# LivGen/LMAT

Measured on AMD Instinct MI355X. Metric: reads/s (150 bp) vs 64 GB k-mer DB, higher is better.
Workload: dtype u64; 1 GPU; 1104000000 x 150 bp reads/GPU vs 64 GiB k-mer hash (6467472668 20-mers, replicated per GPU), run_rl.sh flags -x 0 -j 30 -l 0 -b 1, calls-only; total_reads=1104000000, reads_per_launch=8000000, read_len=150, db_kmers=6467472668, k=20, parallelism=reads sharded x1, DB replicated, genus_block_permille=100, prune_g=0, list_replicas=1, distinct_lists=792576, reads_called=1058323347, read_pool_batches=32

## Files before the change

lmat_amd/csrc/kernels.hip:

```cpp
#include <hip/hip_runtime.h>
#include <atomic>
#include <type_traits>
#include "kernels.hpp"

#ifndef LMAT_ABLATE
#define LMAT_ABLATE 0
#endif
#define STOP_AT(n, v) do { if (LMAT_ABLATE && A.prm.stop_after == (n)) { if (lane == 0) { emit(250, (v)); } return; } } while (0)
#ifndef LMAT_CLOSURE_FAST
#define LMAT_CLOSURE_FAST 1
#endif
#ifndef LMAT_LDS_SHIFT
#define LMAT_LDS_SHIFT 0
#endif

namespace lmat {

#define WSYNC()                                              \
    do {                                                     \
        __builtin_amdgcn_fence(__ATOMIC_SEQ_CST, "wavefront"); \
        __builtin_amdgcn_wave_barrier();                     \
    } while (0)

template <bool GMEM>
// ... 1475 lines not shown
        }
        const bool done = vrow && !bail;
        uint32_t coff = 0, ncand = 0;
        if (A.cands && bal(done && !phix)) {
            uint32_t c0 = 0;
            if (done && !phix && li == 0) c0 = G_ADD(&g_cursor[0], nT);
            coff = bp(c0, 0);
            const bool room = (uint64_t)coff + nT <= A.cand_cap;
            if (done && !phix && !room && li == 0) G_OR((GAS uint32_t*)A.err, (uint32_t)kErrCandOverflow);
            if (done && !phix && room && act)
                ((GAS uint64_t*)((GAS lmat_cand*)A.cands + coff))[nT - 1u - (uint32_t)li] = (uint64_t)g_tid32[ptid] | ((uint64_t)__float_as_uint(pscore) << 32);
            if (room) ncand = nT;
        }
        if (vrow && li == 0) {
            GAS uint64_t* out = (GAS uint64_t*)(A.results + it);
            if (bail) {
                *(GAS uint8_t*)out = 254;
                ((GAS uint32_t*)A.k4_bail)[G_ADD(&g_cursor[6], 1u)] = (uint32_t)it;
            } else {
                lmat_read_result res;
                uint64_t wv[5];
                wv[0] = out[0]; wv[1] = out[1]; wv[2] = out[2]; wv[3] = out[3]; wv[4] = out[4];
                __builtin_memcpy(&res, wv, 40);
                res.cand_kmer_cnt = (uint16_t)cand;
                uint32_t call_idx;
                if (phix) {
                    res.status = LMAT_ST_PHIX; res.match_type = LMAT_MT_DIRECT; res.call_tid = 32630; res.call_score = phix_score;
                    res.log_avg = 0; res.stdev = 0; res.cand_off = 0; res.n_cand = 0;
                    call_idx = A.phix_call_idx;
                } else {
                    res.status = LMAT_ST_CALL; res.match_type = (uint8_t)match; res.log_avg = log_avg; res.stdev = stdev1;
                    res.call_tid = call_tid ? g_tid32[call_tid] : 0u; res.call_score = call_score;
                    res.cand_off = coff; res.n_cand = ncand;
                    call_idx = call_tid;
                }
                store_result(out, res);
                if (res.status != LMAT_ST_PHIX && res.match_type == LMAT_MT_NOMATCH) {
                    G_ADD(&tally_nomatch[1], 1ull);
                } else if (res.call_score >= A.prm.min_score) {
                    G_ADD(&tally_count[call_idx], 1ull);
                    G_ADD(&tally_score[call_idx], (double)res.call_score);
                } else if (res.call_score < A.prm.min_score) {
                    G_ADD(&tally_nomatch[2], 1ull);
                }
            }
        }
    }
}

#define WSYNC_WAVE WSYNC
#pragma push_macro("WSYNC")
#undef WSYNC
#define WSYNC() wsync<(U > 2048)>()
template <int LPR>
__global__ __launch_bounds__(256) void tail_kernel(ClassifyArgs A) {
    const uint64_t gi = (uint64_t)blockIdx.x * 256 + threadIdx.x;
    const uint64_t it = gi / LPR;
    const uint32_t j = (uint32_t)(gi % LPR);
    if (it >= A.count) return;
    const uint64_t r = A.index ? (uint64_t)A.index[it] : A.first + it;
    const DeviceTables& tb = A.tb;
    const int k = tb.k;
    const uint64_t off = A.rec_off[r];
    const uint32_t p = 128u + j;
    const uint32_t wb = (2 * p) >> 5, ws = (2 * p) & 31;
    const uint32_t* codes = A.words + off + 1;
    const uint32_t len = A.words[off], cr0 = codes[wb], cr1 = codes[wb + 1], cr2 = codes[wb + 2];
    if ((int)len < k) return;
    const uint32_t P = len - k + 1;
    if (P <= 128u || P > 128u + LPR) return;
    const uint32_t nb = (len + 15) / 16, nm = (len + 31) / 32;
    const uint32_t* vmask = codes + nb;
    auto cw = [&](uint32_t i) -> uint64_t { const uint32_t v = i == wb ? cr0 : (i == wb + 1 ? cr1 : cr2); return i < nb ? v : 0u; };
    auto vw = [&](uint32_t i) -> uint64_t { return i < nm ? vmask[i] : 0u; };
    const uint64_t kmask = (1ull << (2 * k)) - 1;
    const uint32_t wmask = (1u << k) - 1;
    const uint32_t mb = p >> 5, ms = p & 31;
    const uint64_t m2 = (vw(mb + 1) << 32) | vw(mb);
    const uint64_t lo = (cw(wb + 1) << 32) | cw(wb);
    uint64_t w = ws ? ((lo >> ws) | (cw(wb + 2) << (64 - ws))) : lo;
    w &= kmask;
    const uint64_t rev = (~w) & kmask;
    uint64_t f = __builtin_bitreverse64(w);
    f = ((f & 0x5555555555555555ull) << 1) | ((f >> 1) & 0x5555555555555555ull);
    f >>= (64 - 2 * k);
    const bool fc = f < rev;
    const uint64_t km = fc ? f : rev, kr = fc ? rev : f;
    const uint64_t ri = r - A.result_base;
    if (j < 3u) {
        const int cm = tb.cpt.m;
        const uint64_t x = f >> (2 * (kCptW - 1)), xr = rev & ((1ull << (2 * cm)) - 1);
        ((uint64_t*)A.tail_u)[ri * 4 + j] = (cpt_scramble(x < xr ? x : xr, cm) << 4) | (xr < x ? 2u : 0u) | (x == xr ? 1u : 0u);
    }
    u32x4 e = {0u, 0u, 0u, 0u};
    if (p < P) {
        uint32_t b, tag;
        cpt_address(*(const CptGeom*)&tb.cpt, km, kr, b, tag);
        const uint32_t jj = ((tag - 1u) >> 7) & 3u;
        const uint32_t* bk = (const uint32_t*)tb.slots + (uint64_t)b * 16;
        const u32x4 q0 = *(const u32x4*)bk, q1 = *(const u32x4*)(bk + 4), q2 = *(const u32x4*)(bk + 8), q3 = *(const u32x4*)(bk + 12);
        const uint32_t tg[6] = {q0.x, q0.y, q0.z, q0.w, q1.x, q1.y};
        const uint32_t pw[6] = {q1.z, q1.w, q2.x, q2.y, q2.z, q2.w};
        const uint32_t ph[3] = {q3.x, q3.y, q3.z};
        uint32_t pay = 0;
        bool hit = false;
#pragma unroll
        for (int i = kCptSlots - 1; i >= 0; --i) {
            const uint32_t t = (tg[i >> 1] >> (16 * (i & 1))) & 0xFFFFu;
            if (t == (tag & 0xFFFFu)) {
                hit = true;
                pay = ((pw[i >> 1] >> (16 * (i & 1))) & 0xFFFFu) | (((ph[i >> 2] >> (8 * (i & 3))) & 0xFFu) << 16);
            }
        }
        const bool valid = ((uint32_t)(m2 >> ms) & wmask) == wmask;
        if (valid) {
            if (!hit && (q3.w & kCptOvfFlag)) pay = wide_lookup(tb.ovf_slots, tb.ovf_nbuckets, ovf_bucket_of(b, tag & 0xFFFFu, tb.ovf_nbuckets), km);
            e = u32x4{(uint32_t)km, (uint32_t)(km >> 32), b, pay | (1u << 24) | ((fc ? jj : (uint32_t)(kCptW - 1) - jj) << 30)};
        }
    }
    ((u32x4*)A.tail16)[ri * LPR + j] = e;
}

typedef const ClassifyArgs __attribute__((address_space(4))) CArgs;
template <int U, int T, int E, bool INK4, bool PERM, bool CPT, bool WIDE = false, bool PLAIN = false>
__device__ __forceinline__ void classify_one(CArgs* Ap, uint64_t r, unsigned char* lds, LAS unsigned char* xl, int lane,
                                             const uint32_t* wcur, uint32_t (&nmacc)[2]) {
    using L = WL<U, T, E, INK4, CPT, WIDE>;
    constexpr int THM = L::TH - 1;
    using tid_t = typename std::conditional<WIDE, uint32_t, uint16_t>::type;
    using ent_t = typename std::conditional<WIDE, unsigned long long, unsigned int>::type;
    using lin_t = typename std::conditional<WIDE, LinEntW, LinEnt>::type;
    constexpr int ESH = WIDE ? 32 : 16;
    constexpr ent_t EIDM = WIDE ? (ent_t)0xFFFFFFFFull : (ent_t)0xFFFFu;
    constexpr uint32_t EPEND = WIDE ? 0x80000000u : 0x8000u;
#define RELANE() do { asm volatile("" : "+v"(lane)); } while (0)
#pragma push_macro("A")
#pragma push_macro("tb")
#define A (*Ap)
#define tb (Ap->tb)
    RELANE();
    uint32_t* rd = (uint32_t*)(lds + L::OFF_RD);
    unsigned long long* hv = (unsigned long long*)(lds + L::OFF_R1);
    tid_t* reg = (tid_t*)(lds + L::OFF_R1);
    uint16_t* stamp = (uint16_t*)(reg + T);
    uint16_t* cnt = stamp + T;
    uint16_t* leaf = cnt + T;
    ent_t* hent = (ent_t*)(leaf + T);
    ent_t* best = hent + L::TH;
    uint16_t* dep = (uint16_t*)(best + L::TH);
    uint16_t* ord = dep + T;
    tid_t* tin = (tid_t*)(ord + T);
    tid_t* tout = tin + T;
    float* score = (float*)(tout + T);
    uint8_t* sflags = (uint8_t*)(score + T);
    float* score0 = (float*)(sflags + T);
    float* nm_rp = score0 + T;
    uint8_t* nm_cl = (uint8_t*)(nm_rp + T);
    unsigned long long* ukmer = (unsigned long long*)(lds + L::OFF_R2);
    uint32_t* ubucket = (uint32_t*)(lds + L::OFF_R2 + 8 * U);
    uint32_t* dpay = (uint32_t*)(lds + L::OFF_R2);
    uint16_t* dmult = (uint16_t*)(lds + L::OFF_R2 + 4 * L::D);
    uint16_t* dn = dmult + L::D;
    uint16_t* dstart = dn + L::D;
    uint8_t* dfl = (uint8_t*)(dstart + L::D);
    lin_t* lin = (lin_t*)(lds + L::OFF_R2);
    uint32_t* upay = (uint32_t*)(lds + (CPT ? L::OFF_UPAY_C : L::OFF_R3));
    using eld_t = typename std::conditional<INK4, uint16_t, uint8_t>::type;
    uint32_t* el_poff = (uint32_t*)(lds + L::OFF_R3);
    tid_t* el_t = INK4 ? (tid_t*)(el_poff + E) : (tid_t*)(lds + L::OFF_R3);
    tid_t* el_ta = el_t + E;
    tid_t* el_sp = el_ta + E;
    eld_t* el_d = WIDE ? (eld_t*)(el_sp + E) : (eld_t*)(el_ta + (INK4 ? E : 2 * E));
    uint16_t* el_off = (uint16_t*)(el_ta + E);
// ... 155 lines not shown
    auto cpt_finish = [&](int c, uint64_t km, uint64_t u, uint64_t un, uint64_t fcmask, uint32_t& b_out, uint32_t& t_out) {
        const uint32_t ulo = (uint32_t)u, uhi = (uint32_t)(u >> 32);
        uint32_t u1l, u1h, u2l, u2h, u3l, u3h;
        if constexpr (LSH) {
            const LAS uint64_t* up = (const LAS uint64_t*)xl + c * 64 + lane;
            const uint64_t U1 = up[1], U2 = up[2], U3 = up[3];
            u1l = (uint32_t)U1; u1h = (uint32_t)(U1 >> 32); u2l = (uint32_t)U2; u2h = (uint32_t)(U2 >> 32); u3l = (uint32_t)U3; u3h = (uint32_t)(U3 >> 32);
        } else {
            const int n0l = __builtin_amdgcn_readlane((int)(uint32_t)un, 0), n0h = __builtin_amdgcn_readlane((int)(uint32_t)(un >> 32), 0);
            const int n1l = __builtin_amdgcn_readlane((int)(uint32_t)un, 1), n1h = __builtin_amdgcn_readlane((int)(uint32_t)(un >> 32), 1);
            const int n2l = __builtin_amdgcn_readlane((int)(uint32_t)un, 2), n2h = __builtin_amdgcn_readlane((int)(uint32_t)(un >> 32), 2);
            u1l = (uint32_t)__builtin_amdgcn_update_dpp(n0l, (int)ulo, 0x130, 0xf, 0xf, false);
            u1h = (uint32_t)__builtin_amdgcn_update_dpp(n0h, (int)uhi, 0x130, 0xf, 0xf, false);
            u2l = (uint32_t)__builtin_amdgcn_update_dpp(n1l, (int)u1l, 0x130, 0xf, 0xf, false);
            u2h = (uint32_t)__builtin_amdgcn_update_dpp(n1h, (int)u1h, 0x130, 0xf, 0xf, false);
            u3l = (uint32_t)__builtin_amdgcn_update_dpp(n2l, (int)u2l, 0x130, 0xf, 0xf, false);
            u3h = (uint32_t)__builtin_amdgcn_update_dpp(n2h, (int)u2h, 0x130, 0xf, 0xf, false);
        }
        const bool fc = lane_bit(fcmask);
        const uint32_t dirm = fc ? 0u : 12u;
        const uint64_t a0 = ((uint64_t)uhi << 32) | (ulo + dirm), a1 = ((uint64_t)u1h << 32) | (u1l + (dirm ^ 4u));
        const uint64_t a2 = ((uint64_t)u2h << 32) | (u2l + (dirm ^ 8u)), a3 = ((uint64_t)u3h << 32) | (u3l + (dirm ^ 12u));
        const uint64_t m01 = a0 < a1 ? a0 : a1, m23 = a2 < a3 ? a2 : a3;
        const uint64_t best = m01 < m23 ? m01 : m23;
        const uint32_t j = ((uint32_t)best >> 2) & 3u, fl = (uint32_t)best & 3u;
        const uint32_t strand = fc ? fl >> 1 : (fl == 0u ? 1u : 0u);
        const uint64_t sp = cpt_mix(best >> 4, cm);
        const int lb = PLAIN ? 2 : tb.cpt.lowbits;
        const uint32_t hi = (uint32_t)(sp >> lb), low = (uint32_t)sp & ((1u << lb) - 1);
        const int wsh = tb.cpt.wshift;
        uint32_t b, rho;
        if (wsh >= 0) { b = hi >> wsh; rho = hi & ((1u << wsh) - 1u); }
        else if (wsh == -2) {
            const uint32_t nb32 = (uint32_t)tb.cpt.nb, lowp = hi * nb32;
            const uint64_t nb64 = nb32;
            b = __umulhi(hi, nb32);
            rho = (lowp >= nb32 ? 1u : 0u) + ((uint64_t)lowp >= 2 * nb64 ? 1u : 0u) + ((uint64_t)lowp >= 3 * nb64 ? 1u : 0u);
        }
        else { b = (uint32_t)(((double)hi + 0.5) * tb.cpt.invW); rho = hi - b * tb.cpt.W; }
        const int rs = 2 * (kCptW - 1 - (int)j);
        const uint32_t other = (uint32_t)((km >> (2 * cm + rs)) << rs) | ((uint32_t)km & ((1u << rs) - 1));
        b_out = b;
        t_out = (1u + (((((rho << lb) | low) * 4 + j) * 2 + strand) * 64 + other)) | ((fc ? j : (uint32_t)(kCptW - 1) - j) << 30);
    };
    if (CACHE) {
#pragma unroll
        for (int c = 0; c < CH; ++c) {
            if ((uint32_t)c * 64 >= len) break;
            if (TAILOK && c == 2 && tail_mode()) {
                const uint32_t lpr = PLAIN ? 4u : A.tail_lpr;
                const uint64_t ri = r - A.result_base;
                u32x4 te = {0u, 0u, 0u, 0u};
                uint64_t tu = 0;
                if ((uint32_t)lane < lpr) te = ((const GAS u32x4*)A.tail16)[ri * lpr + lane];
                if (lane < 3) tu = ((const GAS uint64_t*)A.tail_u)[ri * 4 + lane];
                kreg[c] = ((uint64_t)(te.y & 0xFFu) << 32) | te.x;
                hreg[c] = te.z;
                treg[c] = te.w & 0xC0000000u;
                okm[c] = __ballot((te.w >> 24) & 1u);
                valid_kmers += popc64(okm[c]);
                ureg[c] = tu;
                if (128u + (uint32_t)lane < P) upay[128 + lane] = te.w & 0xFFFFFFu;
                continue;
            }
            pass1_chunk((uint32_t)c * 64, kreg[c], hreg[c], treg[c], okm[c], ureg[c], fcm[c]);
        }
        STOP_AT(47, 0);
        if (CPT) {
            if constexpr (LSH) {
                WSYNC();
                LAS uint64_t* ush = (LAS uint64_t*)xl;
#pragma unroll
                for (int c = 0; c < CH; ++c) ush[c * 64 + lane] = ureg[c];
                if (lane < 4) ush[CH * 64 + lane] = 0ull;
                WSYNC();
            }
#pragma unroll
            for (int c = 0; c < CH; ++c) {
                if ((uint32_t)c * 64 >= P) break;
                if (TAILOK && c == 2 && tail_mode()) continue;
                cpt_finish(c, kreg[c], ureg[c], c + 1 < CH ? ureg[c + 1] : 0ull, fcm[c], hreg[c], treg[c]);
            }
        }
    } else {
        for (uint32_t p0 = 0; p0 < len; p0 += 64) { uint64_t a; uint32_t b, t; uint64_t v, u, f; pass1_chunk(p0, a, b, t, v, u, f); }
    }
    WSYNC();
    if (tot > 0) {
        const float q = (float)gc / (float)tot;
        const float gc_pcnt = (float)((double)q * 100.0);
        bin_sel = __builtin_amdgcn_readfirstlane((int)(gc_pcnt / 10.0f));
    }
    if (valid_kmers < A.prm.min_kmer) {
        if (lane == 0) { emit(LMAT_ST_SHORT_VALID, 0); nmacc[0]++; }
        return;
    }
    STOP_AT(1, 0);
    RELANE();
    uint32_t nuniq = 0;
    uint32_t nscan = 0;
    if constexpr (!CPT) {
    auto pass2_chunk = [&](uint32_t p0, uint64_t km, uint32_t h, bool ok) {
        const uint32_t p = p0 + lane;
        const bool first = ok && (uint32_t)(hv[h] & 0xFFFF) == p;
        const uint64_t bm = __ballot(first);
        if (first) {
            const uint32_t rk = nuniq + prefix_count(bm);
            ukmer[rk] = (km << kPayloadBits) + 1;
// ... 1476 lines not shown
            WSYNC();
        }
        if (!done && lane == 0) {
            lmat_read_result res;
            res.status = 255; res.match_type = LMAT_MT_NOMATCH; res.cand_kmer_cnt = 0; res.valid_kmers = 0; res.read_len = 0; res.log_avg = 0;
            res.stdev = 0; res.call_tid = 0; res.call_score = 0; res.cand_off = 0; res.n_cand = 0; res.bin_sel = 0;
            store_result(out, res);
        }
    }
}

template <int LPB>
__global__ __launch_bounds__(64) void gather_bench_kernel(const uint64_t* __restrict__ slots, uint32_t nbuckets,
                                                          uint64_t probes_per_wave, uint64_t seed,
                                                          unsigned long long* sink) {
    const int lane = threadIdx.x & 63, g = lane / LPB, q = lane % LPB;
    constexpr int PPL = 64 / LPB;
    const GAS u32x4* quarters = (const GAS u32x4*)slots;
    unsigned long long acc = 0;
    uint64_t ctr = (uint64_t)blockIdx.x * probes_per_wave;
    for (uint64_t i = 0; i < probes_per_wave; i += 9 * PPL) {
        u32x4 sl[9];
#pragma unroll
        for (int j = 0; j < 9; ++j) {
            uint32_t b = bucket_of(seed + ctr + i + j * PPL + g, nbuckets);
            if (LPB == 8) b &= ~1u;
            sl[j] = quarters[(uint64_t)b * 4 + q];
        }
#pragma unroll
        for (int j = 0; j < 9; ++j) acc += (sl[j].x >> 13) + sl[j].w;
    }
    if (acc == 0x123456789ull) atomicAdd(sink, acc);
}

#pragma push_macro("WSYNC")
#undef WSYNC
#define WSYNC() wsync<(U > 2048)>()
#ifndef LMAT_FAST_WAVES
#define LMAT_FAST_WAVES 8
#endif
constexpr int classify_waves(int U, int E, bool INK4, bool CPT) { return INK4 ? 1 : (E > kFastE ? (U <= 160 ? 5 : 2) : (U <= 160 ? (CPT ? LMAT_FAST_WAVES : 5) : (U <= 256 ? (CPT ? LMAT_FAST_WAVES : 5) : (U <= 320 ? (CPT ? 5 : 3) : (CPT ? 4 : 3))))); }
template <int U, int T, int E, bool INK4, bool PERM, bool CPT, bool WIDE = false, bool PLAIN = false>
__global__ __launch_bounds__(64, classify_waves(U, E, INK4, CPT)) void classify_kernel(ClassifyArgs A) {
    extern __shared__ __align__(16) unsigned char lds_smem[];
    unsigned char* smem = U > 2048 ? A.gscratch + (size_t)blockIdx.x * WL<U, T, E, INK4, false, WIDE>::BYTES : lds_smem;
    LAS unsigned char* xl = (LAS unsigned char*)(U > 2048 ? lds_smem : lds_smem + WL<U, T, E, INK4, CPT, WIDE>::OFF_XL);
    const int lane = threadIdx.x & 63;
    constexpr int NW = (WL<U, T, E, INK4, CPT, WIDE>::RD_WORDS + 1 + 63) / 64;
    const uint32_t G = gridDim.x;
    uint32_t it = blockIdx.x;
    uint32_t wcur[NW], wnext[NW];
    uint32_t nmacc[2] = {0, 0};
    uint64_t off1 = 0;
    {
        const uint64_t count = !PLAIN && A.count_ptr ? (uint64_t)*(const GAS uint32_t*)A.count_ptr : A.count;
        if (it >= count) return;
        const GAS uint32_t* index = PLAIN ? nullptr : (const GAS uint32_t*)A.index;
        const GAS uint64_t* rec_off = (const GAS uint64_t*)A.rec_off;
        const GAS uint32_t* words = (const GAS uint32_t*)A.words;
        auto r_of = [&](uint64_t i) -> uint64_t { return index ? (uint64_t)index[i] : A.first + i; };
        const uint64_t off0 = rec_off[r_of(it)];
        off1 = (uint64_t)it + G < count ? rec_off[r_of((uint64_t)it + G)] : 0;
#pragma unroll
        for (int j = 0; j < NW; ++j) wcur[j] = words[off0 + lane + 64 * j];
    }
    while (true) {
        CArgs* Ap = (CArgs*)__builtin_amdgcn_kernarg_segment_ptr();
        asm volatile("" : "+s"(Ap));
        const uint64_t count = !PLAIN && Ap->count_ptr ? (uint64_t)*(const GAS uint32_t*)Ap->count_ptr : Ap->count;
        const GAS uint32_t* index = PLAIN ? nullptr : (const GAS uint32_t*)Ap->index;
        const GAS uint64_t* rec_off = (const GAS uint64_t*)Ap->rec_off;
        const GAS uint32_t* words = (const GAS uint32_t*)Ap->words;
        auto r_of = [&](uint64_t i) -> uint64_t { return index ? (uint64_t)index[i] : Ap->first + i; };
        const uint64_t off2 = (uint64_t)it + 2 * (uint64_t)G < count ? rec_off[r_of((uint64_t)it + 2 * (uint64_t)G)] : 0;
        const bool more = (uint64_t)it + G < count;
#pragma unroll
        for (int j = 0; j < NW; ++j) wnext[j] = more ? words[off1 + lane + 64 * j] : 0u;
        classify_one<U, T, E, INK4, PERM, CPT, WIDE, PLAIN>(Ap, r_of(it), smem, xl, lane, wcur, nmacc);
        WSYNC();
#pragma unroll
        for (int j = 0; j < NW; ++j) wcur[j] = wnext[j];
        off1 = off2;
        if (!more) break;
        it += G;
    }
    if (lane == 0) {
        GAS unsigned long long* tally_nomatch = (GAS unsigned long long*)A.counts + 2 * (uint64_t)A.tb.n_ids;
        if (nmacc[0]) G_ADD(&tally_nomatch[0], (unsigned long long)nmacc[0]);
        if (nmacc[1]) G_ADD(&tally_nomatch[1], (unsigned long long)nmacc[1]);
    }
}

#pragma pop_macro("WSYNC")

struct PerDeviceOnce {
    std::atomic<unsigned char> done[64];
    PerDeviceOnce() { for (auto& d : done) d.store(0); }
    template <class F> void operator()(F&& f) {
        int dev = 0;
        if (hipGetDevice(&dev) != hipSuccess || dev < 0 || dev >= 64) { f(); return; }
        if (!done[dev].load(std::memory_order_acquire)) { f(); done[dev].store(1, std::memory_order_release); }
    }
};

static int grid_for(uint64_t n, int per_block, int cap) {
    uint64_t b = (n + per_block - 1) / per_block;
    if (b < 1) b = 1;
    if (b > (uint64_t)cap) b = cap;
    return (int)b;
}

__global__ __launch_bounds__(256) void fill_offsets_kernel(uint64_t* __restrict__ off, uint64_t* __restrict__ rec_off, uint64_t n,
                                                           uint32_t len, uint32_t words_per_rec) {
    const uint64_t i = (uint64_t)blockIdx.x * 256 + threadIdx.x;
    if (i <= n) { off[i] = i * len; rec_off[i] = i * words_per_rec; }
}
void launch_fill_offsets(uint64_t* off, uint64_t* rec_off, uint64_t n, uint32_t len, hipStream_t stream) {
    fill_offsets_kernel<<<dim3((unsigned)((n + 1 + 255) / 256)), dim3(256), 0, stream>>>(off, rec_off, n, len, rec_words(len));
}
void launch_pack_reads(const uint8_t* bases, const uint64_t* off, const uint64_t* rec_off, uint32_t* words, uint64_t n,
                       hipStream_t stream) {
    hipLaunchKernelGGL(pack_reads_kernel, dim3(grid_for(n, 16, 16384)), dim3(256), 0, stream, bases, off, rec_off, words, n);
}
void launch_insert_pairs(const DeviceTables& tb, const uint64_t* kmers, const uint32_t* payload, uint64_t n,
                         uint32_t* fail, hipStream_t stream) {
    hipLaunchKernelGGL(insert_pairs_kernel, dim3(grid_for(n, 256, 16384)), dim3(256), 0, stream, tb, kmers, payload, n, fail);
}
void launch_synth_db(const DeviceTables& tb, const SynthGeo& g, int k, const uint16_t* strain_idx, const uint32_t* list_payload,
// ... 81 lines not shown
        k4_kernel<false, kK4MidT, 64><<<dim3((unsigned)g2), dim3(64), 0, stream2>>>(b);
    }
    hipStreamWaitEvent(stream3, forked, 0);
    if (!a.nm.active && a.prm.k4_row) {
        uint64_t gr = (a.count + 3) / 4;
        if (gr > 256 * 64) gr = 256 * 64;
        if (gr < 1) gr = 1;
        k4_row_kernel<<<dim3((unsigned)gr), dim3(64), 0, stream3>>>(a);
    }
    if (!a.nm.active) launch_k4_lds<kK4T>(a, a.count / 8 + 64, stream3);
    if (small_stream != stream && small_stream != stream3) hipStreamWaitEvent(small_stream, forked, 0);
    launch_k4_lds<kK4SmallT>(a, a.count, small_stream);
}
void launch_k4_end(const ClassifyArgs& a, hipStream_t join_stream, hipStream_t stream2, hipStream_t stream3, hipStream_t small_stream,
                   hipEvent_t joined2, hipEvent_t joined3, hipEvent_t joined_small, hipEvent_t done) {
    if (stream2 != join_stream) { hipEventRecord(joined2, stream2); hipStreamWaitEvent(join_stream, joined2, 0); }
    if (stream3 != join_stream) { hipEventRecord(joined3, stream3); hipStreamWaitEvent(join_stream, joined3, 0); }
    if (small_stream != join_stream && small_stream != stream3 && small_stream != stream2) {
        hipEventRecord(joined_small, small_stream);
        hipStreamWaitEvent(join_stream, joined_small, 0);
    }
    ClassifyArgs b = a;
    b.k4_slot = kCurK4Bail;
    if (a.nm.active) k4_kernel<true, kK4T, 64><<<dim3(64), dim3(64), 0, join_stream>>>(b);
    else k4_kernel<false, kK4T, 64><<<dim3(64), dim3(64), 0, join_stream>>>(b);
    hipEventRecord(done, join_stream);
}

static int k4_static_of(const ClassifyArgs& a) {
    const int stop = a.prm.stop_after;
    const bool base = !a.nm.active && a.tb.depth_consistent && !(a.cands && !a.prm.prn_all);
    const bool wave = base && (stop == 0 || (stop >= 30 && stop <= 34));
    const bool rows = base && a.prm.k4_row && stop == 0;
    return (wave ? 1 : 0) | (rows ? 2 : 0);
}
static bool plain_launch(const ClassifyArgs& a, int k4_static) {
    static const bool on = !LMAT_ABLATE && (!getenv("LMAT_PLAIN") || atoi(getenv("LMAT_PLAIN")) != 0);
    return on && a.tb.k == 20 && a.tb.cpt.nb && a.tb.cpt.m == 17 && a.tb.cpt.lowbits == 2 && !a.tb.wide && !a.nm.active && !a.rand_max &&
           !a.gene_mode && !a.prm.permissive && a.prm.stop_after == 0 && k4_static == 1 && !a.cands && a.prm.hbias == 0.0f &&
           a.p_min == 0 && a.p_max == 0xFFFFFFFFu && !a.index && !a.count_ptr && a.tail_lpr == 4;
}
static std::atomic<unsigned long long> g_variant_launches[64][2];
void classify_variant_launches(int device, uint64_t out[2]) {
    out[0] = out[1] = 0;
    if (device < 0 || device >= 64) return;
    out[0] = g_variant_launches[device][0].load();
    out[1] = g_variant_launches[device][1].load();
}
template <int U, int T, int E, bool INK4, bool PERM, bool CPT, bool WIDE = false, bool PLAIN = false>
static void launch_classify_t(const ClassifyArgs& a_in, hipStream_t stream) {
    using L = WL<U, T, E, INK4, CPT, WIDE>;
    ClassifyArgs a = a_in;
    a.prm.k4_static = k4_static_of(a);
    constexpr bool kPlainClass = U == 160 && T == 64 && E == kFastE && !INK4 && !PERM && CPT && !WIDE;
    if constexpr (kPlainClass && !PLAIN && !LMAT_ABLATE) {
        if (plain_launch(a, a.prm.k4_static)) { launch_classify_t<U, T, E, INK4, PERM, CPT, WIDE, true>(a_in, stream); return; }
    }
    if constexpr (kPlainClass) {
        int dev = 0;
        if (hipGetDevice(&dev) == hipSuccess && dev >= 0 && dev < 64) g_variant_launches[dev][PLAIN ? 1 : 0]++;
    }
    if (U > 2048) {
        int grid = kGmemGrid;
        if (!a.count_ptr && (uint64_t)grid > a.count) grid = (int)(a.count ? a.count : 1);
        classify_kernel<U, T, E, INK4, PERM, CPT, WIDE><<<dim3(grid), dim3(64), CPT ? L::XL_BYTES : 0, stream>>>(a);
        return;
    }
    static const int lds_pad = getenv("LMAT_LDS_PAD") ? atoi(getenv("LMAT_LDS_PAD")) : 0;
    const int lds_bytes = L::BYTES + lds_pad;
    static PerDeviceOnce attr_once;
    attr_once([lds_bytes] { hipFuncSetAttribute((const void*)classify_kernel<U, T, E, INK4, PERM, CPT, WIDE, PLAIN>, hipFuncAttributeMaxDynamicSharedMemorySize, lds_bytes); });
    const int per_cu = 160 * 1024 / lds_bytes;
    static const int gmult = getenv("LMAT_GRID_MULT") ? atoi(getenv("LMAT_GRID_MULT")) : 32;
    int grid = 256 * (per_cu < 1 ? 1 : (per_cu > 32 ? 32 : per_cu)) * (gmult > 0 ? gmult : 32);
    if (!a.count_ptr && (uint64_t)grid > a.count) grid = (int)a.count;
    if (a.count_ptr && INK4 && grid > 256 * (per_cu < 2 ? 2 : per_cu)) grid = 256 * (per_cu < 2 ? 2 : per_cu);
    if (grid < 1) grid = 1;
    classify_kernel<U, T, E, INK4, PERM, CPT, WIDE, PLAIN><<<dim3(grid), dim3(64), lds_bytes, stream>>>(a);
}

void launch_k4_debug(const ClassifyArgs& a, const uint32_t* idx, const float* scores, const uint64_t* off, const float* stdevs, uint64_t n,
                     hipStream_t stream) {
    if (!n) return;
    k4_debug_kernel<<<dim3((unsigned)((n + 63) / 64)), dim3(64), 0, stream>>>(a, idx, scores, off, stdevs, n);
}

void launch_k4_debug_counts(const ClassifyArgs& a, const uint32_t* idx, const uint32_t* cnts, const uint64_t* off, const uint32_t* cands, uint64_t n,
                            bool on_the_wave, hipStream_t stream) {
    if (!n) return;
    if (on_the_wave) {
        const uint64_t g = n < 256 * 32 ? n : 256 * 32;
        ClassifyArgs b = a;
        b.prm.k4_static = k4_static_of(b);
        k4_wave_debug_kernel<<<dim3((unsigned)g), dim3(64), 0, stream>>>(b, idx, cnts, off, cands, n);
    } else k4_debug_counts_kernel<<<dim3((unsigned)((n + 63) / 64)), dim3(64), 0, stream>>>(a, idx, cnts, off, cands, n);
}

void launch_tail(const ClassifyArgs& a, hipStream_t stream) {
    if (!a.tail_lpr || !a.count || a.count_ptr) return;
    const uint64_t lanes = a.count * a.tail_lpr;
    const dim3 grid((unsigned)((lanes + 255) / 256));
    if (a.tail_lpr == 4) tail_kernel<4><<<grid, dim3(256), 0, stream>>>(a);
    else if (a.tail_lpr == 8) tail_kernel<8><<<grid, dim3(256), 0, stream>>>(a);
    else tail_kernel<16><<<grid, dim3(256), 0, stream>>>(a);
}

int classify_max_read_len() { return kGmemU + 19; }
size_t classify_gmem_scratch_bytes() { return (size_t)kGmemGrid * WL<kGmemU, 4096, 16384, true, false, true>::BYTES; }

#define LC(U, T, E, K)                                                                                                   \
    (a.tb.cpt.nb ? (a.prm.permissive ? launch_classify_t<U, T, E, K, true, true>(a, stream) : launch_classify_t<U, T, E, K, false, true>(a, stream)) \
                 : (a.prm.permissive ? launch_classify_t<U, T, E, K, true, false>(a, stream) : launch_classify_t<U, T, E, K, false, false>(a, stream)))
#define LCW(U, T, E) (a.prm.permissive ? launch_classify_t<U, T, E, true, true, true, true>(a, stream) : launch_classify_t<U, T, E, true, false, true, true>(a, stream))
bool launch_classify(const ClassifyArgs& a, uint32_t max_read_len, int tcap_class, hipStream_t stream) {
    const int k = a.tb.k;
    const uint32_t P = max_read_len >= (uint32_t)k ? max_read_len - k + 1 : 0;
    if (a.tb.wide) {
        if (!a.tb.cpt.nb) return false;
        if (tcap_class == 4) { if (P > 512) return false; LCW(512, 128, 512); }
        else if (tcap_class == 5) { if (P <= 512) LCW(512, 512, 2048); else if (P <= 2048) LCW(2048, 512, 2048); else return false; }
        else if (P <= (uint32_t)kGmemU && a.gscratch) LCW(kGmemU, 4096, 16384);
        else return false;
        return true;
    }
    if (tcap_class == 2) {
        if (P <= 160) LC(160, 64, 512, false); else LC(512, 64, 512, false);
    } else if (tcap_class == 3) {
        if (P > 512) return false;
        LC(512, 256, 1024, true);
    } else if (P <= 160 && tcap_class == 0) {
        LC(160, 64, kFastE, false);
    } else if (P <= 256) {
        if (tcap_class == 0) LC(256, 64, kFastE, false); else LC(256, 1024, 4096, true);
    } else if (P <= 320 && tcap_class == 0) {
        LC(320, 64, kFastE, false);
    } else if (P <= 512) {
        if (tcap_class == 0) LC(512, 64, kFastE, false); else LC(512, 1024, 4096, true);
    } else if (P <= 2048) {
        LC(2048, 1024, 4096, true);
    } else if (P <= (uint32_t)kGmemU && a.gscratch) {
        LC(kGmemU, 4096, 16384, true);
    } else {
        return false;
    }
    return true;
}

uint32_t synth_strain_base_host(const SynthGeo& g, uint32_t species, uint32_t strain_global, uint64_t pos) {
    return synth_strain_base(g, species, strain_global, pos);
}
void synth_window_host(const SynthGeo& g, int k, uint32_t species, uint64_t pos, uint64_t* kmer, uint32_t* first_strain, uint32_t* mask, bool* inblk,
                       int* cons_level) {
// ... 63 lines not shown
```

lmat_amd/csrc/kernels.hpp:

```cpp
#pragma once
#include "lmat_internal.hpp"

namespace lmat {

struct ClassifyArgs {
    DeviceTables tb;
    KernelParams prm;
    const uint32_t* words;
    const uint64_t* rec_off;
    const uint32_t* index;
    uint32_t p_min = 0, p_max = 0xFFFFFFFFu;
    uint64_t first, count;
    uint64_t result_base;
    lmat_read_result* results;
    lmat_cand* cands;
    uint64_t cand_cap;
    uint32_t* cursor;
    uint32_t cand_chunk = 0;
    uint32_t cand_sub_mask = 0;
    uint32_t* err;
    void* counts;
    uint32_t phix_call_idx;
    uint32_t* ovf_list;
    uint32_t ovf_slot;
    const uint32_t* count_ptr;
    uint32_t* k4buf;
    uint32_t* k4_small;
    uint32_t* k4_mid;
    uint32_t* k4_large;
    uint32_t* k4_bail;
    uint32_t* k4_row;
    uint32_t k4_slot;
    uint32_t* rand_max;
    uint32_t* rand_cnt;
    const uint8_t* rand_gc;
    uint32_t rand_nb;
    unsigned char* gscratch;
    NullModelDev nm;
    uint32_t gene_mode = 0;
    const uint32_t* tail16 = nullptr;
    const uint64_t* tail_u = nullptr;
    uint32_t tail_lpr = 0;
};

static const int kK4T = 64;
static const int kK4RecWords = 2 + kK4T;

static const int kCandSubs = 1024;
static const int kCursorWords = 16;
static const size_t kCursorBytes = kCursorWords * 4 + (size_t)kCandSubs * 64;
enum CursorWord {
    kCurCand = 0,
    kCurOvfFast = 2,
    kCurOvfE512 = 3,
    kCurOvfMid = 10,
    kCurOvfLarge = 7,
    kCurK4Small = 4,
    kCurK4Large = 5,
    kCurK4Mid = 8,
    kCurK4Row = 9,
    kCurK4Bail = 6,
    kCurBatchErr = 15,
};

enum { kErrTidOverflow = 1, kErrReadTooLong = 2, kErrCandOverflow = 4, kErrLineageTrunc = 8, kErrNoNullModel = 16 };

void launch_fill_offsets(uint64_t* off, uint64_t* rec_off, uint64_t n, uint32_t len, hipStream_t stream);
void launch_pack_reads(const uint8_t* bases, const uint64_t* off, const uint64_t* rec_off, uint32_t* words, uint64_t n,
                       hipStream_t stream);
void launch_insert_pairs(const DeviceTables& tb, const uint64_t* kmers, const uint32_t* payload, uint64_t n,
                         uint32_t* fail, hipStream_t stream);
void launch_synth_db(const DeviceTables& tb, const SynthGeo& g, int k, const uint16_t* strain_idx, const uint32_t* list_payload,
                     uint64_t g_off, uint32_t rep, uint32_t rep_stride, uint32_t* fail, unsigned long long* inserted, hipStream_t stream);
void launch_table_count(const DeviceTables& tb, unsigned long long* out, hipStream_t stream);
void launch_synth_reads(uint32_t* words, const uint64_t* rec_off, const uint32_t* lengths, uint32_t n_lengths, uint64_t n,
                        uint64_t seed, const SynthGeo& g, hipStream_t stream);
void launch_lookup(const DeviceTables& tb, const uint64_t* kmers, uint64_t n, uint32_t* counts, uint32_t* tids,
                   uint32_t stride, hipStream_t stream);
void launch_div_check(unsigned long long* out2, hipStream_t stream);
void launch_probe_stats(const DeviceTables& tb, const uint64_t* kmers, uint64_t n, unsigned long long* out, hipStream_t stream);
void launch_tail(const ClassifyArgs& a, hipStream_t stream);
bool launch_classify(const ClassifyArgs& a, uint32_t max_read_len, int tcap_class, hipStream_t stream);
void launch_k4_begin(const ClassifyArgs& a, hipStream_t stream, hipStream_t stream2, hipStream_t stream3, hipStream_t small_stream,
                     hipEvent_t forked);
void launch_k4_end(const ClassifyArgs& a, hipStream_t join_stream, hipStream_t stream2, hipStream_t stream3, hipStream_t small_stream,
                   hipEvent_t joined2, hipEvent_t joined3, hipEvent_t joined_small, hipEvent_t done);
void launch_k4_debug(const ClassifyArgs& a, const uint32_t* idx, const float* scores, const uint64_t* off, const float* stdevs, uint64_t n,
                     hipStream_t stream);
void launch_k4_debug_counts(const ClassifyArgs& a, const uint32_t* idx, const uint32_t* cnts, const uint64_t* off, const uint32_t* cands, uint64_t n,
                            bool on_the_wave, hipStream_t stream);
void classify_variant_launches(int device, uint64_t out[2]);
int classify_max_read_len();
size_t classify_gmem_scratch_bytes();
void launch_gather_bench(const uint64_t* slots, uint32_t nbuckets, uint64_t n_probes, uint64_t seed,
                         unsigned long long* sink, hipStream_t stream, int bytes_per_probe = 64);
// ... 10 lines not shown
```

lmat_amd/csrc/lmat_api.cpp:

```cpp
#include <hip/hip_runtime.h>
#include <algorithm>
#include <cmath>
#include <cstdio>
#include <cstring>
#include <chrono>
#include <string>
#include <thread>
#include <atomic>
#include <fcntl.h>
#include <unistd.h>
#include "kernels.hpp"
#include "outfmt.hpp"

using namespace lmat;

#define HIPCHK(ctx, call)                                                                          \
    do {                                                                                           \
        hipError_t e__ = (call);                                                                   \
        if (e__ != hipSuccess)                                                                     \
            return set_err(ctx, LMAT_E_DEVICE, std::string(#call) + ": " + hipGetErrorString(e__)); \
    } while (0)

template <class T>
static int dev_upload(lmat_ctx* c, T** dst, const std::vector<T>& src) {
// ... 1289 lines not shown
    a.cursor = s.word(0);
    a.err = c->batch_err ? s.word(kCurBatchErr) : c->d_err;
    a.counts = c->out_counts ? c->out_counts : c->d_counts;
    auto it = c->tax.index_of.find(32630);
    a.phix_call_idx = it == c->tax.index_of.end() ? 0 : it->second;
    a.ovf_list = s.ovf[0].as<uint32_t>();
    a.ovf_slot = kCurOvfFast;
    a.count_ptr = nullptr;
    a.k4buf = s.k4buf.as<uint32_t>();
    a.gscratch = nullptr;
    a.rand_max = nullptr;
    a.rand_cnt = nullptr;
    a.rand_gc = nullptr;
    a.rand_nb = 0;
    if (c->rand_launch) { a.rand_max = c->d_rand_max; a.rand_cnt = c->d_rand_cnt; a.rand_gc = c->rand_gc.as<uint8_t>(); a.rand_nb = c->rand_nb; }
    a.k4_small = s.k4small.as<uint32_t>();
    a.k4_large = s.k4large.as<uint32_t>();
    a.k4_mid = a.k4_large + s.scratch_reads;
    a.k4_row = a.k4_large + 2 * s.scratch_reads;
    a.k4_bail = s.k4bail.as<uint32_t>();
    a.k4_slot = kCurK4Large;
    a.nm = c->nm;
    a.gene_mode = (uint32_t)c->gene_mode;
    if (c->gene_mode) a.prm.min_kmer = 0;
    return a;
}

static bool pipeline_on() {
    static const bool on = !getenv("LMAT_PIPELINE") || atoi(getenv("LMAT_PIPELINE")) != 0;
    return on;
}

static int err_read_too_long(lmat_ctx* c) {
    return set_err(c, LMAT_E_CAPACITY, "read longer than " + std::to_string(classify_max_read_len()) + " bases");
}


static int prepare_set(lmat_ctx* c, uint64_t count, bool want_cands, uint64_t cand_cap, bool pipelined) {
    if (pipelined) c->cur_set ^= 1;
    BatchSet& s = c->set();
    if (!s.done) HIPCHK(c, hipEventCreateWithFlags(&s.done, hipEventDisableTiming));
    if (s.in_flight) HIPCHK(c, hipStreamWaitEvent(c->stream, s.done, 0));
    int rc = ensure_results(c, s, c->out_results ? 0 : count, want_cands && !c->out_cands ? cand_cap : 0);
    if (!rc) rc = ensure_scratch(c, s, count);
    if (rc) return rc;
    HIPCHK(c, c->gscratch.ensure(classify_gmem_scratch_bytes()));
    HIPCHK(c, hipMemsetAsync(s.cursor.p, 0, want_cands ? kCursorBytes : (size_t)kCursorWords * 4, c->stream));
    return LMAT_OK;
}

static void plan_tail(lmat_ctx* c, BatchSet& s, const lmat_reads* reads, bool single_class, ClassifyArgs& a) {
    static const bool tail_on = !getenv("LMAT_TAIL") || atoi(getenv("LMAT_TAIL")) != 0;
    static const int tail_force = getenv("LMAT_TAIL_LPR") ? atoi(getenv("LMAT_TAIL_LPR")) : 0;
    const uint32_t k = (uint32_t)c->dev.k;
    const uint32_t realP = reads->max_len >= k ? reads->max_len - k + 1 : 0;
    if (single_class && realP > 160u) return;
    const uint32_t maxP = std::min<uint32_t>(realP, 160u);
    uint32_t lpr = 0;
    if (tail_on && c->dev.cpt.nb && !c->nm.active && maxP > 128u) lpr = maxP <= 132u ? 4u : (maxP <= 136u ? 8u : 16u);
    if (lpr && (tail_force == 4 || tail_force == 8 || tail_force == 16) && 128u + (uint32_t)tail_force >= std::min(maxP, 144u)) lpr = (uint32_t)tail_force;
    if (!lpr) return;
    if (s.tail.ensure(a.count * (16ull * lpr + 32ull)) != hipSuccess) { (void)hipGetLastError(); return; }
    a.tail_lpr = lpr;
    a.tail16 = s.tail.as<uint32_t>();
    a.tail_u = (const uint64_t*)(s.tail.as<unsigned char>() + a.count * 16ull * lpr);
}

static int build_class_lists(lmat_ctx* c, lmat_reads* rw) {
    const uint32_t k = (uint32_t)c->dev.k;
    if (rw->preset || rw->cls_k == (int)k || rw->lens.size() != rw->n) return LMAT_OK;
    for (int j = 0; j < kNCls; ++j) { rw->cls_host[j].clear(); if (rw->cls_dev[j]) { hipFree(rw->cls_dev[j]); rw->cls_dev[j] = nullptr; } }
    for (uint64_t i = 0; i < rw->n; ++i) {
        const uint32_t P = rw->lens[i] >= k ? rw->lens[i] - k + 1 : 0;
        rw->cls_host[len_class(P)].push_back((uint32_t)i);
    }
    int used = 0;
    for (int j = 0; j < kNCls; ++j) used += !rw->cls_host[j].empty();
    if (used > 1)
        for (int j = 0; j < kNCls; ++j)
            if (!rw->cls_host[j].empty()) {
                HIPCHK(c, hipMalloc((void**)&rw->cls_dev[j], rw->cls_host[j].size() * 4));
                HIPCHK(c, hipMemcpyAsync(rw->cls_dev[j], rw->cls_host[j].data(), rw->cls_host[j].size() * 4, hipMemcpyHostToDevice, c->stream));
            }
    rw->cls_k = (int)k;
    return LMAT_OK;
}

struct ClassSpan { const uint32_t* index; uint64_t count; uint32_t max_len; bool tail; };
static int class_spans(const lmat_ctx* c, const lmat_reads* r, uint64_t first, uint64_t count, ClassSpan out[kNCls]) {
    const uint32_t k = (uint32_t)c->dev.k;
    const bool mixed = r->cls_dev[0] || r->cls_dev[1] || r->cls_dev[2] || r->cls_dev[3];
    int n = 0;
    for (int j = 0; j < kNCls; ++j) {
        uint64_t lo = 0, hi = 0;
        if (r->preset) hi = r->cls_n[j];
        else if (mixed) {
            const std::vector<uint32_t>& v = r->cls_host[j];
            lo = std::lower_bound(v.begin(), v.end(), (uint32_t)first) - v.begin();
            hi = std::lower_bound(v.begin(), v.end(), (uint32_t)(first + count)) - v.begin();
        }
        if (hi > lo) out[n++] = ClassSpan{r->cls_dev[j] + lo, hi - lo, kClsU[j] + k - 1, j == 0};
    }
    if (r->preset ? n > 1 : mixed) return n;
    out[0] = ClassSpan{nullptr, count, std::min<uint32_t>(r->max_len, 512 + k - 1), true};
    return 1;
}

struct LaunchEvents {
    hipEvent_t e[4] = {nullptr, nullptr, nullptr, nullptr};
    bool timed = false, started = false;
    ~LaunchEvents() { for (hipEvent_t x : e) if (x) hipEventDestroy(x); }
    void start(hipStream_t st) {
        if (timed && !started) hipEventRecord(e[0], st);
        started = true;
    }
};
// ... 837 lines not shown
```

Baseline: 382.8 million reads/s.

## Fuse tail k-mer lookup into classify kernel instead of separate tail launch

Moves the tail-position k-mer hashing and bucket probe (positions 128..128+LPR) out of a separate pre-pass kernel and into the main classify kernel. Every 64/lpr trips, a wave computes tail entries for 64/lpr upcoming reads and stores them to global memory. Consumers later read those entries back with relaxed agent-scope atomic loads after a workgroup fence. This saves one kernel launch and a full grid pass per batch, at the cost of extra latency and divergence inside the main loop, plus a subtle cross-wave visibility dependency.

New measurement: 385.1 million reads/s, median of 6. No clear change (+0.6%).

```diff
diff --git a/lmat_amd/csrc/kernels.hip b/lmat_amd/csrc/kernels.hip
--- a/lmat_amd/csrc/kernels.hip
+++ b/lmat_amd/csrc/kernels.hip
@@ -1551,25 +1551,20 @@
 #pragma push_macro("WSYNC")
 #undef WSYNC
 #define WSYNC() wsync<(U > 2048)>()
-template <int LPR>
-__global__ __launch_bounds__(256) void tail_kernel(ClassifyArgs A) {
-    const uint64_t gi = (uint64_t)blockIdx.x * 256 + threadIdx.x;
-    const uint64_t it = gi / LPR;
-    const uint32_t j = (uint32_t)(gi % LPR);
-    if (it >= A.count) return;
-    const uint64_t r = A.index ? (uint64_t)A.index[it] : A.first + it;
-    const DeviceTables& tb = A.tb;
+template <class AR>
+__device__ __forceinline__ void tail_lane(AR& A, uint64_t r, uint32_t j, uint32_t lpr) {
+    const auto& tb = A.tb;
     const int k = tb.k;
-    const uint64_t off = A.rec_off[r];
+    const uint64_t off = ((const GAS uint64_t*)A.rec_off)[r];
     const uint32_t p = 128u + j;
     const uint32_t wb = (2 * p) >> 5, ws = (2 * p) & 31;
-    const uint32_t* codes = A.words + off + 1;
-    const uint32_t len = A.words[off], cr0 = codes[wb], cr1 = codes[wb + 1], cr2 = codes[wb + 2];
+    const GAS uint32_t* codes = (const GAS uint32_t*)A.words + off + 1;
+    const uint32_t len = codes[-1], cr0 = codes[wb], cr1 = codes[wb + 1], cr2 = codes[wb + 2];
     if ((int)len < k) return;
     const uint32_t P = len - k + 1;
-    if (P <= 128u || P > 128u + LPR) return;
+    if (P <= 128u || P > 128u + lpr) return;
     const uint32_t nb = (len + 15) / 16, nm = (len + 31) / 32;
-    const uint32_t* vmask = codes + nb;
+    const GAS uint32_t* vmask = codes + nb;
     auto cw = [&](uint32_t i) -> uint64_t { const uint32_t v = i == wb ? cr0 : (i == wb + 1 ? cr1 : cr2); return i < nb ? v : 0u; };
     auto vw = [&](uint32_t i) -> uint64_t { return i < nm ? vmask[i] : 0u; };
     const uint64_t kmask = (1ull << (2 * k)) - 1;
@@ -1589,15 +1584,15 @@
     if (j < 3u) {
         const int cm = tb.cpt.m;
         const uint64_t x = f >> (2 * (kCptW - 1)), xr = rev & ((1ull << (2 * cm)) - 1);
-        ((uint64_t*)A.tail_u)[ri * 4 + j] = (cpt_scramble(x < xr ? x : xr, cm) << 4) | (xr < x ? 2u : 0u) | (x == xr ? 1u : 0u);
+        ((GAS uint64_t*)A.tail_u)[ri * 4 + j] = (cpt_scramble(x < xr ? x : xr, cm) << 4) | (xr < x ? 2u : 0u) | (x == xr ? 1u : 0u);
     }
     u32x4 e = {0u, 0u, 0u, 0u};
     if (p < P) {
         uint32_t b, tag;
         cpt_address(*(const CptGeom*)&tb.cpt, km, kr, b, tag);
         const uint32_t jj = ((tag - 1u) >> 7) & 3u;
-        const uint32_t* bk = (const uint32_t*)tb.slots + (uint64_t)b * 16;
-        const u32x4 q0 = *(const u32x4*)bk, q1 = *(const u32x4*)(bk + 4), q2 = *(const u32x4*)(bk + 8), q3 = *(const u32x4*)(bk + 12);
+        const GAS uint32_t* bk = (const GAS uint32_t*)tb.slots + (uint64_t)b * 16;
+        const u32x4 q0 = *(const GAS u32x4*)bk, q1 = *(const GAS u32x4*)(bk + 4), q2 = *(const GAS u32x4*)(bk + 8), q3 = *(const GAS u32x4*)(bk + 12);
         const uint32_t tg[6] = {q0.x, q0.y, q0.z, q0.w, q1.x, q1.y};
         const uint32_t pw[6] = {q1.z, q1.w, q2.x, q2.y, q2.z, q2.w};
         const uint32_t ph[3] = {q3.x, q3.y, q3.z};
@@ -1617,7 +1612,14 @@
             e = u32x4{(uint32_t)km, (uint32_t)(km >> 32), b, pay | (1u << 24) | ((fc ? jj : (uint32_t)(kCptW - 1) - jj) << 30)};
         }
     }
-    ((u32x4*)A.tail16)[ri * LPR + j] = e;
+    ((GAS u32x4*)A.tail16)[ri * lpr + j] = e;
+}
+template <int LPR>
+__global__ __launch_bounds__(256) void tail_kernel(ClassifyArgs A) {
+    const uint64_t gi = (uint64_t)blockIdx.x * 256 + threadIdx.x;
+    const uint64_t it = gi / LPR;
+    if (it >= A.count) return;
+    tail_lane(A, A.index ? (uint64_t)A.index[it] : A.first + it, (uint32_t)(gi % LPR), (uint32_t)LPR);
 }
 
 typedef const ClassifyArgs __attribute__((address_space(4))) CArgs;
@@ -1879,8 +1881,13 @@
                 const uint64_t ri = r - A.result_base;
                 u32x4 te = {0u, 0u, 0u, 0u};
                 uint64_t tu = 0;
-                if ((uint32_t)lane < lpr) te = ((const GAS u32x4*)A.tail16)[ri * lpr + lane];
-                if (lane < 3) tu = ((const GAS uint64_t*)A.tail_u)[ri * 4 + lane];
+                auto ld = [](const GAS uint64_t* p) -> uint64_t { return __hip_atomic_load(p, __ATOMIC_RELAXED, __HIP_MEMORY_SCOPE_AGENT); };
+                if ((uint32_t)lane < lpr) {
+                    const GAS uint64_t* tp = (const GAS uint64_t*)A.tail16 + (ri * lpr + lane) * 2;
+                    const uint64_t t0 = ld(tp), t1 = ld(tp + 1);
+                    te = u32x4{(uint32_t)t0, (uint32_t)(t0 >> 32), (uint32_t)t1, (uint32_t)(t1 >> 32)};
+                }
+                if (lane < 3) tu = ld((const GAS uint64_t*)A.tail_u + ri * 4 + lane);
                 kreg[c] = ((uint64_t)(te.y & 0xFFu) << 32) | te.x;
                 hreg[c] = te.z;
                 treg[c] = te.w & 0xC0000000u;
@@ -3463,6 +3470,7 @@
     uint32_t wcur[NW], wnext[NW];
     uint32_t nmacc[2] = {0, 0};
     uint64_t off1 = 0;
+    uint32_t trip = 0;
     {
         const uint64_t count = !PLAIN && A.count_ptr ? (uint64_t)*(const GAS uint32_t*)A.count_ptr : A.count;
         if (it >= count) return;
@@ -3485,6 +3493,18 @@
         auto r_of = [&](uint64_t i) -> uint64_t { return index ? (uint64_t)index[i] : Ap->first + i; };
         const uint64_t off2 = (uint64_t)it + 2 * (uint64_t)G < count ? rec_off[r_of((uint64_t)it + 2 * (uint64_t)G)] : 0;
         const bool more = (uint64_t)it + G < count;
+        if constexpr (CPT && U == 160 && !INK4) {
+            const uint32_t lpr = PLAIN ? (Ap->tail_wave ? 4u : 0u) : Ap->tail_wave;
+            if (lpr) {
+                const uint32_t lsh = (uint32_t)__builtin_ctz(lpr);
+                if ((trip & ((64u >> lsh) - 1u)) == 0u) {
+                    const uint64_t i = (uint64_t)it + (uint64_t)((uint32_t)lane >> lsh) * G;
+                    if (i < count) tail_lane(*Ap, r_of(i), (uint32_t)lane & (lpr - 1u), lpr);
+                    __builtin_amdgcn_fence(__ATOMIC_ACQ_REL, "workgroup");
+                }
+            }
+            ++trip;
+        }
 #pragma unroll
         for (int j = 0; j < NW; ++j) wnext[j] = more ? words[off1 + lane + 64 * j] : 0u;
         classify_one<U, T, E, INK4, PERM, CPT, WIDE, PLAIN>(Ap, r_of(it), smem, xl, lane, wcur, nmacc);
@@ -3672,6 +3692,7 @@
     using L = WL<U, T, E, INK4, CPT, WIDE>;
     ClassifyArgs a = a_in;
     a.prm.k4_static = k4_static_of(a);
+    if (a.count_ptr || a.tail_wave != a.tail_lpr) a.tail_wave = 0;
     constexpr bool kPlainClass = U == 160 && T == 64 && E == kFastE && !INK4 && !PERM && CPT && !WIDE;
     if constexpr (kPlainClass && !PLAIN && !LMAT_ABLATE) {
         if (plain_launch(a, a.prm.k4_static)) { launch_classify_t<U, T, E, INK4, PERM, CPT, WIDE, true>(a_in, stream); return; }
@@ -3717,7 +3738,7 @@
 }
 
 void launch_tail(const ClassifyArgs& a, hipStream_t stream) {
-    if (!a.tail_lpr || !a.count || a.count_ptr) return;
+    if (!a.tail_lpr || !a.count || a.count_ptr || a.tail_wave) return;
     const uint64_t lanes = a.count * a.tail_lpr;
     const dim3 grid((unsigned)((lanes + 255) / 256));
     if (a.tail_lpr == 4) tail_kernel<4><<<grid, dim3(256), 0, stream>>>(a);
diff --git a/lmat_amd/csrc/kernels.hpp b/lmat_amd/csrc/kernels.hpp
--- a/lmat_amd/csrc/kernels.hpp
+++ b/lmat_amd/csrc/kernels.hpp
@@ -41,6 +41,7 @@
     const uint32_t* tail16 = nullptr;
     const uint64_t* tail_u = nullptr;
     uint32_t tail_lpr = 0;
+    uint32_t tail_wave = 0;
 };
 
 static const int kK4T = 64;
diff --git a/lmat_amd/csrc/lmat_api.cpp b/lmat_amd/csrc/lmat_api.cpp
--- a/lmat_amd/csrc/lmat_api.cpp
+++ b/lmat_amd/csrc/lmat_api.cpp
@@ -1365,6 +1365,7 @@
 static void plan_tail(lmat_ctx* c, BatchSet& s, const lmat_reads* reads, bool single_class, ClassifyArgs& a) {
     static const bool tail_on = !getenv("LMAT_TAIL") || atoi(getenv("LMAT_TAIL")) != 0;
     static const int tail_force = getenv("LMAT_TAIL_LPR") ? atoi(getenv("LMAT_TAIL_LPR")) : 0;
+    static const bool tail_wave = !getenv("LMAT_TAIL_WAVE") || atoi(getenv("LMAT_TAIL_WAVE")) != 0;
     const uint32_t k = (uint32_t)c->dev.k;
     const uint32_t realP = reads->max_len >= k ? reads->max_len - k + 1 : 0;
     if (single_class && realP > 160u) return;
@@ -1375,6 +1376,7 @@
     if (!lpr) return;
     if (s.tail.ensure(a.count * (16ull * lpr + 32ull)) != hipSuccess) { (void)hipGetLastError(); return; }
     a.tail_lpr = lpr;
+    a.tail_wave = tail_wave ? lpr : 0u;
     a.tail16 = s.tail.as<uint32_t>();
     a.tail_u = (const uint64_t*)(s.tail.as<unsigned char>() + a.count * 16ull * lpr);
 }
```
